# TorontoDeepLearning/convnet

Hardware: AMD Instinct MI355X
Metric: images/sec (fprop+bprop+wgrad) AlexNet 224x224 bs=256 (higher is better)
Workload: dtype f32

## Files before the change

convnet_amd/csrc/elementwise.hip:

```cpp
#include <cfloat>
#include <climits>
#include <cmath>

#include "common.h"

namespace chip {

using f32x4 = __attribute__((ext_vector_type(4))) float;

constexpr int kThreads = 256;
constexpr int kMaxBlocks = 2048;

inline int blocks_for(size_t work_items) {
  size_t b = (work_items + kThreads - 1) / kThreads;
  if (b > kMaxBlocks) b = kMaxBlocks;
  if (b < 1) b = 1;
  return (int)b;
}

template <typename F>
__global__ void map2_kernel(float* __restrict__ out, const float* a, const float* b, size_t n, bool vec, F f) {
  const size_t tid = (size_t)blockIdx.x * blockDim.x + threadIdx.x, stride = (size_t)gridDim.x * blockDim.x;
  if (vec) {
    const size_t n4 = n >> 2;
// ... 201 lines not shown
      const float b = mult * vec[(i << 2) / rows];
      f32x4 v = reinterpret_cast<const f32x4*>(mat)[i];
      v = v + b;
      reinterpret_cast<f32x4*>(out)[i] = v;
    }
  } else {
    for (size_t i = tid; i < n; i += stride) out[i] = mat[i] + mult * vec[i / rows];
  }
}

int add_row(cudamat* mat, cudamat* vec, cudamat* target, float mult) {
  if (!mat->on_device || !vec->on_device || !target->on_device) return ERROR_NOT_ON_DEVICE;
  if (mat->is_trans) return ERROR_TRANSPOSED;
  if (mat->size[1] != vec->size[1] || vec->size[0] != 1 || mat->size[0] != target->size[0] || mat->size[1] != target->size[1])
    return ERROR_INCOMPATIBLE_DIMENSIONS;
  const size_t n = numel(mat);
  const bool v4 = (mat->size[0] & 3) == 0 && aligned16(mat->data_device) && aligned16(target->data_device);
  hipLaunchKernelGGL(add_row_kernel, dim3(blocks_for(n / 4 + 1)), dim3(kThreads), 0, stream(), target->data_device, mat->data_device,
                     vec->data_device, mat->size[0], n, mult, v4);
  return launch_status();
}

__device__ __forceinline__ void sgd_one(float& g, float& w, float& h, float l2, float clip, float eps, float mom);

template <bool DO_SGD>
__global__ void rows_sq_kernel(float* __restrict__ g, float* __restrict__ w, float* __restrict__ h, int rows, int cols, int chunk,
                               float* __restrict__ partial, float l2, float clip, float eps, float mom) {
  const int r = blockIdx.x * blockDim.x + threadIdx.x;
  if (r >= rows) return;
  const int c0 = blockIdx.y * chunk, c1 = min(cols, c0 + chunk);
  float s = 0.f;
  for (int c = c0; c < c1; ++c) {
    const size_t i = (size_t)r + (size_t)rows * c;
    float wv = w[i];
    if (DO_SGD) {
      float gv = g[i], hv = h[i];
      sgd_one(gv, wv, hv, l2, clip, eps, mom);
      g[i] = gv;
      h[i] = hv;
      w[i] = wv;
    }
    s += wv * wv;
  }
  partial[(size_t)blockIdx.y * rows + r] = s;
}

template <bool DO_SGD>
__global__ void rows_sq4_kernel(float* __restrict__ g, float* __restrict__ w, float* __restrict__ h, int rows, int cols, int chunk,
                                float* __restrict__ partial, float l2, float clip, float eps, float mom) {
  const int r = 4 * (blockIdx.x * blockDim.x + threadIdx.x);
  if (r >= rows) return;
  const int c0 = blockIdx.y * chunk, c1 = min(cols, c0 + chunk);
  f32x4 s = {0.f, 0.f, 0.f, 0.f};
  auto one = [&](int c) {
    const size_t i = (size_t)r + (size_t)rows * c;
    f32x4 wv = *reinterpret_cast<f32x4*>(w + i);
    if (DO_SGD) {
      f32x4 gv = *reinterpret_cast<f32x4*>(g + i), hv = *reinterpret_cast<f32x4*>(h + i);
#pragma unroll
      for (int e = 0; e < 4; ++e) {
        float a = gv[e], b = wv[e], d = hv[e];
        sgd_one(a, b, d, l2, clip, eps, mom);
        gv[e] = a; wv[e] = b; hv[e] = d;
      }
      *reinterpret_cast<f32x4*>(g + i) = gv;
      *reinterpret_cast<f32x4*>(h + i) = hv;
      *reinterpret_cast<f32x4*>(w + i) = wv;
    }
    s += wv * wv;
  };
  int c = c0;
  for (; c + 1 < c1; c += 2) {
    one(c);
    one(c + 1);
  }
  if (c < c1) one(c);
  *reinterpret_cast<f32x4*>(partial + (size_t)blockIdx.y * rows + r) = s;
}

__global__ void row_factor_kernel(const float* __restrict__ partial, int nchunks, int rows, float norm, int constraint, float* __restrict__ factor) {
  __shared__ float sh[4][64];
  const int r = blockIdx.x * 64 + (threadIdx.x & 63), q = threadIdx.x >> 6;
  float s = 0.f;
  if (r < rows)
    for (int k = q; k < nchunks; k += 4) s += partial[(size_t)k * rows + r];
  sh[q][threadIdx.x & 63] = s;
  __syncthreads();
  if (q != 0 || r >= rows) return;
  s = sqrtf((sh[0][threadIdx.x] + sh[1][threadIdx.x]) + (sh[2][threadIdx.x] + sh[3][threadIdx.x]));
  factor[r] = (constraint == 1 || s > norm) ? norm / s : 1.f;
}

__global__ void row_scale_kernel(const float* __restrict__ src, float* __restrict__ dst, int rows, int cols, int chunk, const float* __restrict__ factor) {
  const int r = blockIdx.x * blockDim.x + threadIdx.x;
  const float f = r < rows ? factor[r] : 1.f;
  const bool in_place = src == dst;
  if (in_place && !__syncthreads_or(f != 1.f)) return;
  if (r >= rows) return;
  const int c0 = blockIdx.y * chunk, c1 = min(cols, c0 + chunk);
  for (int c = c0; c < c1; ++c) {
    const size_t i = (size_t)r + (size_t)rows * c;
    dst[i] = src[i] * f;
  }
}

inline int rows_normlimit(float* g, float* w_in, float* w_out, float* h, int rows, int cols, float norm, int constraint, bool do_sgd,
                          float l2, float clip, float eps, float mom) {
  int chunk = 64;
  while ((long)divup(rows, 256) * divup(cols, chunk) > 4096 && chunk < cols) chunk *= 2;
  const int nchunks = divup(cols, chunk);
  float* partial = static_cast<float*>(workspace(sizeof(float) * ((size_t)nchunks * rows + rows)));
  float* factor = partial + (size_t)nchunks * rows;
  dim3 grid(divup(rows, 256), nchunks);
  const bool v4 = (rows & 3) == 0 && aligned16(w_in) && (!do_sgd || (aligned16(g) && aligned16(h)));
  KernelTimer timer(do_sgd ? "rows_sq_kernel<sgd> + row_scale_kernel" : "rows_sq_kernel + row_scale_kernel", do_sgd ? "sgd_normlimit" : "normlimit", 0.0,
                    4.0 * (double)rows * cols * (do_sgd ? 7 : 3));
  if (v4) {
    const dim3 g4(divup(rows / 4, 64), nchunks);
    if (do_sgd)
      hipLaunchKernelGGL(rows_sq4_kernel<true>, g4, dim3(64), 0, stream(), g, w_in, h, rows, cols, chunk, partial, l2, clip, eps, mom);
    else
      hipLaunchKernelGGL(rows_sq4_kernel<false>, g4, dim3(64), 0, stream(), nullptr, w_in, nullptr, rows, cols, chunk, partial, 0.f, 0.f, 0.f, 0.f);
  } else if (do_sgd)
    hipLaunchKernelGGL(rows_sq_kernel<true>, grid, dim3(256), 0, stream(), g, w_in, h, rows, cols, chunk, partial, l2, clip, eps, mom);
  else
    hipLaunchKernelGGL(rows_sq_kernel<false>, grid, dim3(256), 0, stream(), nullptr, w_in, nullptr, rows, cols, chunk, partial, 0.f, 0.f, 0.f, 0.f);
  hipLaunchKernelGGL(row_factor_kernel, dim3(divup(rows, 64)), dim3(256), 0, stream(), partial, nchunks, rows, norm, constraint, factor);
  hipLaunchKernelGGL(row_scale_kernel, grid, dim3(256), 0, stream(), w_in, w_out, rows, cols, chunk, factor);
  return launch_status();
// ... 918 lines not shown
```

convnet_amd/csrc/gather_gemm.hip:

```cpp
#include <algorithm>
#include <array>
#include <cmath>
#include <map>
#include <vector>
#include <cstdlib>
#include <string>
#include <type_traits>

#include "common.h"

#include "gather_gemm.h"

namespace chip {

template <int WR, int WC, int MT, int CW, bool A_KCONTIG, bool VEC, bool O3 = false, bool SPLIT = false>
__global__ __launch_bounds__(WR* WC * 64, (O3 ? 3 : 2)) void gg_kernel(const GGParams pin, const GGClassTable ct) {
  constexpr int NT = WR * WC * 64;
  constexpr int NTC = CW / 32, CW4 = CW / 4;
  using fvec = __attribute__((ext_vector_type(NTC))) float;
  constexpr int ROWS = WR * MT * 32;
  constexpr int APITCH = A_KCONTIG ? (BK + 4) : ROWS;
  constexpr int A_STAGE = A_KCONTIG ? ROWS * APITCH : BK * ROWS;
  constexpr int B_STAGE = WC * BK * CW;
  constexpr int NA = ((A_KCONTIG ? ROWS * (BK / 4) : BK * (ROWS / 4)) + NT - 1) / NT;
// ... 733 lines not shown
#pragma unroll
    for (int t = 0; t < MT; ++t) a[0][t] = ar[lh * ROWS + t * 32];
    b4[0] = *reinterpret_cast<const fvec*>(bs + lh * BROW);
    static_for<0, BK / 2>([&](auto KK) __attribute__((always_inline)) {
      constexpr int kk = decltype(KK)::value;
      constexpr int cur = kk & 1, nxt = cur ^ 1;
      if constexpr (kk + 1 < BK / 2) {
        const int krow = 2 * (kk + 1) + lh;
#pragma unroll
        for (int t = 0; t < MT; ++t) a[nxt][t] = ar[krow * ROWS + t * 32];
        b4[nxt] = *reinterpret_cast<const fvec*>(bs + krow * BROW);
      }
      __builtin_amdgcn_sched_barrier(0);
#pragma unroll
      for (int t = 0; t < MT; ++t)
#pragma unroll
        for (int u = 0; u < NTC; ++u)
          acc[t][u] = __builtin_amdgcn_mfma_f32_32x32x2f32(a[cur][t], b4[cur][u], acc[t][u], 0, 0, 0);
    });
    stage = stage == ST - 1 ? 0 : stage + 1;
    __syncthreads();
  }

  if (tsplit >= 0) {
    float* pp = p.tail_partial + ((size_t)(L - p.tail_first) * p.tail_splits + tsplit) * (size_t)(ROWS * WC * CW);
#pragma unroll
    for (int t = 0; t < MT; ++t)
#pragma unroll
      for (int reg = 0; reg < 16; ++reg) {
        fvec v;
#pragma unroll
        for (int u = 0; u < NTC; ++u) v[u] = acc[t][u][reg];
        *reinterpret_cast<fvec*>(pp + ((size_t)(t * 16 + reg) * NC + tid) * NTC) = v;
      }
    return;
  }
  gg_epilogue<WR, WC, MT, CW, true>(p, acc, row_tile, col_tile, split, T.ncols, T.GX, T.G, T.dy0, T.dx0);
}

__global__ void gg_reduce_kernel(float* __restrict__ dst, const float* __restrict__ partial, const float* __restrict__ bias,
                                 size_t total, size_t slab, int splits, size_t per_row, float scaleTargets, int relu,
                                 const float* __restrict__ mask, float post_scale) {
  for (size_t i = (size_t)blockIdx.x * blockDim.x + threadIdx.x; i < total; i += (size_t)gridDim.x * blockDim.x) {
    float s = 0.f;
    for (int k = 0; k < splits; ++k) s += partial[(size_t)k * slab + i];
    if (scaleTargets != 0.f) s = scaleTargets * dst[i] + s;
    if (bias) s += bias[i / per_row];
    if (relu) s = s > 0.f ? s : 0.f;
    if (mask) s = mask[i] > 0.f ? s * post_scale : 0.f;
    dst[i] = s;
  }
}

__global__ void dgrad_filter_kernel(const float* __restrict__ W, float* __restrict__ Wt, int F, int C, int Ky, int Kx, int cy,
                                    int cx, int sy, int sx, int TYc, int TXc, int tap_major) {
  const size_t total = (size_t)C * TXc * TYc * F;
  for (size_t i = (size_t)blockIdx.x * blockDim.x + threadIdx.x; i < total; i += (size_t)gridDim.x * blockDim.x) {
    const int c = i % C;
    size_t r = i / C;
    int a, b, f;
    if (tap_major) {
      const int f16 = r % 16;
      r /= 16;
      const int tap = r % (TXc * TYc);
      const int fb = r / (TXc * TYc);
      f = fb * 16 + f16;
      a = tap / TXc;
      b = tap - a * TXc;
    } else {
      b = r % TXc;
      r /= TXc;
      a = r % TYc;
      f = r / TYc;
    }
    Wt[i] = W[(size_t)f + (size_t)F * ((cx + sx * b) + Kx * ((cy + sy * a) + Ky * c))];
  }
}

__global__ void filter_tapmajor_kernel(const float* __restrict__ W, float* __restrict__ Wt, int F, int C, int TYX) {
  const size_t total = (size_t)F * C * TYX;
  for (size_t i = (size_t)blockIdx.x * blockDim.x + threadIdx.x; i < total; i += (size_t)gridDim.x * blockDim.x) {
    const int f = i % F;
    size_t r = i / F;
    const int c16 = r % 16;
    r /= 16;
    const int tap = r % TYX;
    const int c = (int)(r / TYX) * 16 + c16;
    Wt[i] = W[(size_t)f + (size_t)F * (tap + (size_t)TYX * c)];
  }
}

template <int WM, int WN, int MT, int NTL, bool VEC, int TS, bool SPLIT = false>
__global__ __launch_bounds__(WM* WN * 64) void wg_kernel(const WGParams p) {
  constexpr int NT = WM * WN * 64;
  constexpr int KT = WM * MT * TS;
  constexpr int FT = WN * NTL * TS;
  constexpr int LH = 64 / TS;
  using facc = __attribute__((ext_vector_type(TS == 32 ? 16 : 4))) float;
  constexpr int PITCH = VEC ? WG_NB : WG_PITCH;
  constexpr int A_STAGE = KT * PITCH, B_STAGE = FT * PITCH;
  constexpr int NA = (KT * 8 + NT - 1) / NT, NB = (FT * 8 + NT - 1) / NT;
  extern __shared__ __attribute__((aligned(16))) float smem[];
  float* As = smem;
  float* Bs = smem + 2 * A_STAGE;

  const int tiles = p.k_tiles * p.f_tiles;
// ... 250 lines not shown
        if (fin) {
          v = v * p.scaleOutput;
          if (p.scaleTargets != 0.f) v = p.scaleTargets * ld4(dp) + v;
        }
        st4(dp, v);
      }
      return;
    }
  }
#pragma unroll
  for (int u = 0; u < NTL; ++u) {
    const int f = f0 + (wn * NTL + u) * TS + li;
    if (f >= p.F) continue;
#pragma unroll
    for (int t = 0; t < MT; ++t) {
#pragma unroll
      for (int reg = 0; reg < (TS == 32 ? 16 : 4); ++reg) {
        const int k = kc0 + (wm * MT + t) * TS + (TS == 32 ? (reg & 3) + 8 * (reg >> 2) + 4 * lh : 4 * lh + reg);
        if (k >= KB) continue;
        float* dp = (fin && k == p.K) ? p.bias_dst + f : out + (size_t)k * p.F + f;
        float v = acc[t][u][reg];
        if (fin) {
          v *= p.scaleOutput;
          if (p.scaleTargets != 0.f) v = p.scaleTargets * (*dp) + v;
        }
        *dp = v;
      }
    }
  }
}

__global__ void wg_reduce_group_kernel(float* __restrict__ stage, const float* __restrict__ partial, size_t total, int splits, int per) {
  const int g = blockIdx.y;
  const int k0 = g * per, k1 = min(splits, k0 + per);
  for (size_t i = (size_t)blockIdx.x * blockDim.x + threadIdx.x; i < total; i += (size_t)gridDim.x * blockDim.x) {
    float s = 0.f;
    for (int k = k0; k < k1; ++k) s += partial[(size_t)k * total + i];
    stage[(size_t)g * total + i] = s;
  }
}

__global__ void wg_reduce_kernel(float* __restrict__ dst, float* __restrict__ dst2, const float* __restrict__ partial, size_t total,
                                 size_t main, int splits, float scaleTargets, float scaleOutput) {
  for (size_t i = (size_t)blockIdx.x * blockDim.x + threadIdx.x; i < total; i += (size_t)gridDim.x * blockDim.x) {
    float s = 0.f;
    for (int k = 0; k < splits; ++k) s += partial[(size_t)k * total + i];
    s *= scaleOutput;
    float* d = i < main ? dst + i : dst2 + (i - main);
    if (scaleTargets != 0.f) s = scaleTargets * (*d) + s;
    *d = s;
  }
}

__global__ void __launch_bounds__(256) dot_generic_kernel(const float* __restrict__ a, const float* __restrict__ b, float* __restrict__ c, int m, int n,
                                                          int k, int ld1, int ld2, int t1, int t2, float beta, float alpha) {
  __shared__ float As[32][33], Bs[32][33];
  const int tx = threadIdx.x & 31, ty = threadIdx.x >> 5;
  const int i0 = blockIdx.x * 32, j0 = blockIdx.y * 32;
  float acc[4] = {0.f, 0.f, 0.f, 0.f};
  for (int l0 = 0; l0 < k; l0 += 32) {
    for (int r = ty; r < 32; r += 8) {
      if (t1) {
        const int i = i0 + r, l = l0 + tx;
        As[tx][r] = (i < m && l < k) ? a[(size_t)l + (size_t)ld1 * i] : 0.f;
      } else {
        const int i = i0 + tx, l = l0 + r;
        As[r][tx] = (i < m && l < k) ? a[(size_t)i + (size_t)ld1 * l] : 0.f;
      }
      if (t2) {
        const int j = j0 + tx, l = l0 + r;
        Bs[r][tx] = (j < n && l < k) ? b[(size_t)j + (size_t)ld2 * l] : 0.f;
      } else {
        const int j = j0 + r, l = l0 + tx;
        Bs[tx][r] = (j < n && l < k) ? b[(size_t)l + (size_t)ld2 * j] : 0.f;
      }
    }
    __syncthreads();
#pragma unroll 8
    for (int l = 0; l < 32; ++l) {
      const float av = As[l][tx];
#pragma unroll
      for (int q = 0; q < 4; ++q) acc[q] = fmaf(av, Bs[l][ty + 8 * q], acc[q]);
    }
    __syncthreads();
  }
  const int i = i0 + tx;
  if (i < m) {
#pragma unroll
    for (int q = 0; q < 4; ++q) {
      const int j = j0 + ty + 8 * q;
      if (j < n) {
        float* d = c + (size_t)i + (size_t)m * j;
        *d = (beta != 0.f ? beta * (*d) : 0.f) + alpha * acc[q];
      }
    }
  }
}

namespace {

constexpr int kTargetBlocks = 512;

struct GGTimer {
  const char* op;
  double flops, exec;
};
// ... 159 lines not shown
  int slots = o3 ? 768 : kTargetBlocks;
  if constexpr (kHasProducer<WC, CW, AK>) {
    if (p.KC > 0) slots = ggp_slots<WR, WC, MT, CW>(gg_split_mode(), p.apre != 0);
  }
  const double block_rate = gg_split_mode() ? 190e12 / slots : 64.0 * 4 * 2.2e9 * 0.8 / 2;
  const double flops = 2.0 * ROWS * (WC * (double)CW) * (double)p.K;
  const bool may_tail = dst_elems > 0 && gg_partial_last_round(tiles, slots, kchunks) && !CHIP_DIAG_KNOB("CONVNET_GG_NO_TAIL_SPLIT", 0);
  double best_t = 1e30;
  int splits = gg_split_k(tiles, slots, flops, block_rate, dst_elems, kchunks, kchunks, &best_t);
  int tail_s_instead = 0;
  if (splits > 1 && may_tail) {
    const int full = (tiles / slots) * slots, rem = tiles - full;
    const double t_round = flops / block_rate, tile_bytes = sizeof(float) * (double)ROWS * WC * CW;
    for (int s = 2; s <= 8 && kchunks / s >= 8; ++s) {
      const double t = (full / (double)slots + std::ceil(rem * (double)s / (double)slots) / s) * t_round + rem * (s + 1.0) * tile_bytes / 4.0e12 + 6e-6;
      if (t < best_t) {
        splits = 1;
        tail_s_instead = s;
        break;
      }
    }
  }
  p.chunks_per_split = kchunks > 0 ? divup(kchunks, splits) : 1;
  splits = kchunks > 0 ? divup(kchunks, p.chunks_per_split) : 1;
  p.splits = splits;
  p.slab = dst_elems;
  p.partial = splits > 1 ? static_cast<float*>(workspace(sizeof(float) * dst_elems * splits)) : nullptr;
  p.tail_splits = 1;
  p.tail_partial = nullptr;
  if (splits == 1 && may_tail) {
    int best_s = gg_tail_split(tiles, slots, flops, block_rate, TILE, kchunks);
    if (best_s == 1 && tail_s_instead > 1) best_s = tail_s_instead;
    if (best_s > 1) gg_set_tail(p, tiles, slots, kchunks, best_s, TILE);
  }
  dim3 grid(p.tail_splits > 1 ? 8 * (p.tail_tf8 + p.tail_tt8) : ((tiles + 7) / 8) * 8, splits);
  gg_launch_variant<WR, WC, MT, CW, AK>(p, kNoClasses, vec, o3, grid, lds_pad, tm);
  if (p.tail_splits > 1) {
    const int rem = tiles - p.tail_first;
    KernelTimer timer("gg_tail_fix_kernel", tm.op, 0.0, sizeof(float) * (double)rem * (p.tail_splits + 1) * ROWS * WC * CW);
    if (vec) hipLaunchKernelGGL((gg_tail_fix_kernel<WR, WC, MT, CW, true>), dim3(rem * kTailFixParts), dim3(WR * WC * 64), 0, stream(), p);
    else hipLaunchKernelGGL((gg_tail_fix_kernel<WR, WC, MT, CW, false>), dim3(rem * kTailFixParts), dim3(WR * WC * 64), 0, stream(), p);
  }
  if (splits > 1) gg_reduce_launch(p, dst_elems, splits, tm.op);
}

}

void wg_reduce_launch(const WGParams& p, size_t total, int splits, int groups, const char* op) {
  KernelTimer timer("wg_reduce_kernel", op, 0.0, sizeof(float) * (double)total * (splits + 1));
  size_t nb = (total + 255) / 256;
  if (nb > 4096) nb = 4096;
  const float* slabs = p.partial;
  int nslabs = splits;
  if (groups > 1) {
    float* stage = p.partial + (size_t)splits * total;
    const int per = divup(splits, groups);
    hipLaunchKernelGGL(wg_reduce_group_kernel, dim3((unsigned)nb, divup(splits, per)), dim3(256), 0, stream(), stage, p.partial, total, splits, per);
    slabs = stage;
    nslabs = divup(splits, per);
  }
  hipLaunchKernelGGL(wg_reduce_kernel, dim3((unsigned)nb), dim3(256), 0, stream(), p.dst, p.bias_dst, slabs, total, (size_t)p.K * p.F, nslabs,
                     p.scaleTargets, p.scaleOutput);
}

namespace {
struct WGBatch {
  int frames = 0, frame = 0, splits = 0;
  size_t total = 0;
  void* (*arena)(size_t) = nullptr;
  size_t max_bytes = 0;
  WGParams last;
};
WGBatch g_wgb;
}
void wg_batch_begin(int frames, void* (*slab_arena)(size_t), size_t max_bytes) {
  g_wgb = WGBatch{};
  g_wgb.frames = frames;
  g_wgb.arena = slab_arena;
  g_wgb.max_bytes = max_bytes;
}
bool wg_batch_active() { return g_wgb.frames > 0; }
int wg_batch_frame() { return g_wgb.frame; }
float* wg_batch_partial(const WGParams& p, size_t total, int splits) {
  WGBatch& b = g_wgb;
  if (!b.frames) return nullptr;
  CHIP_REQUIRE(b.frame < b.frames);
  const size_t S = (size_t)b.frames * splits;
  const size_t bytes = sizeof(float) * total * (S + (S > 64 ? 32 : 0));
  if (b.frame == 0) {
    if (bytes > b.max_bytes) {
      b.frames = 0;
      return nullptr;
    }
    b.splits = splits;
    b.total = total;
  }
  CHIP_REQUIRE(b.splits == splits && b.total == total);
  float* arena = static_cast<float*>(b.arena(bytes));
  b.last = p;
  b.last.partial = arena;
  return arena + (size_t)b.frame++ * splits * total;
}
void wg_batch_end() {
  WGBatch& b = g_wgb;
  if (b.frames && b.frame > 0) {
    CHIP_REQUIRE(b.frame == b.frames);
    const int S = b.frames * b.splits;
    wg_reduce_launch(b.last, b.total, S, S > 64 ? 32 : 1, "conv_wgrad");
  }
  b.frames = 0;
}

void gg_reduce_launch(const GGParams& p, size_t dst_elems, int splits, const char* op) {
  KernelTimer timer("gg_reduce_kernel", op, 0.0, sizeof(float) * (double)dst_elems * (splits + 1));
  size_t nb = (dst_elems + 255) / 256;
  if (nb > 4096) nb = 4096;
  hipLaunchKernelGGL(gg_reduce_kernel, dim3((unsigned)nb), dim3(256), 0, stream(), p.dst, p.partial, p.bias, dst_elems, p.slab, splits,
                     (size_t)p.DP * p.N, p.scaleTargets, p.relu, p.mask, p.post_scale);
}

namespace {

template <bool AK>
void gg_run(GGParams& p, bool vec, size_t dst_elems, const GGTimer& tm) {
  gg_with_tile(gg_tile(p.R, vec, p.skinny != 0), [&](auto t) {
    using T = decltype(t);
    gg_launch_cfg<T::WR, T::WC, T::MT, T::CW, AK>(p, vec, dst_elems, tm);
  });
}

void gg_run_classes(GGParams& p, GGClassTable& ct, bool vec, const GGTimer& tm) {
  gg_with_tile(gg_tile(p.R, vec, false), [&](auto t) {
    using T = decltype(t);
    gg_launch_classes<T::WR, T::WC, T::MT, T::CW>(p, ct, vec, tm);
  });
}

template <int WM, int WN, int MT, int NTL, int TS = 32>
void wg_launch_cfg(WGParams& p, bool vec, const GGTimer& tm) {
  constexpr int KT = WM * MT * TS, FT = WN * NTL * TS;
  const size_t lds = sizeof(float) * 2 * (KT + FT) * (vec ? WG_NB : WG_PITCH);
  p.k_tiles = divup(p.K, KT);
  if (p.bias_dst && divup(p.K + 1, KT) != p.k_tiles) p.bias_dst = nullptr;
  p.f_tiles = divup(p.F, FT);
  p.zero = zero_page();
  p.prio = wg_prio_mode();
  const int tiles = p.k_tiles * p.f_tiles;
  const size_t total = (size_t)(p.K + (p.bias_dst ? 1 : 0)) * p.F;
  const bool no_wide = CHIP_DIAG_KNOB("CONVNET_WG_NO_WIDE", 0) != 0;
  p.wide = (!no_wide && vec && TS == 32 && WM == 2 && WN == 2 && MT == 2 && NTL == 2 && p.F % 4 == 0 && aligned16(p.dst) &&
            (!p.bias_dst || aligned16(p.bias_dst))) ? 1 : 0;
  int splits = 1;
  if (tiles < kTargetBlocks) {
    splits = kTargetBlocks / tiles;
    const int max_by_len = p.chunks_total / 16 > 0 ? p.chunks_total / 16 : 1;
    if (splits > max_by_len) splits = max_by_len;
    const size_t max_by_bytes = (size_t(256) << 20) / (total * sizeof(float)) + 1;
    if ((size_t)splits > max_by_bytes) splits = (int)max_by_bytes;
    if (splits > 1024) splits = 1024;
    if (splits < 1) splits = 1;
  }
  p.chunks_per_split = divup(p.chunks_total, splits);
  splits = divup(p.chunks_total, p.chunks_per_split);
  p.splits = splits;
  const int groups = splits > 64 ? 32 : 1;
  float* const frame_slabs = wg_batch_partial(p, total, splits);
  p.partial = frame_slabs ? frame_slabs
                          : splits > 1 ? static_cast<float*>(workspace(sizeof(float) * total * (splits + (groups > 1 ? groups : 0)))) : nullptr;
  dim3 grid(((tiles * splits + 7) / 8) * 8), block(WM * WN * 64);
  static const std::string kname_f = "wg_kernel<" + std::to_string(WM) + "," + std::to_string(WN) + "," + std::to_string(MT) + "," + std::to_string(NTL) + (TS == 16 ? ",x16>" : ">");
  static const std::string kname_s = kname_f.substr(0, kname_f.size() - 1) + ",split>";
// ... 451 lines not shown
```

convnet_amd/csrc/pool_norm.hip:

```cpp
#include <cfloat>
#include <cstdlib>
#include <mutex>
#include <utility>

#include "common.h"

namespace chip {

using f32x4 = __attribute__((ext_vector_type(4))) float;

struct PoolGeo {
  int N, C, H, W, Ky, Kx, sy, sx, py, px, My, Mx;
  int nvec;
  int xper, xtotal, xrows, xbx;
};

__device__ __forceinline__ bool pool_block(const PoolGeo& g, int& bx, int& row, int& c) {
  if (g.xper == 0) {
    bx = blockIdx.x; row = blockIdx.y; c = blockIdx.z;
    return true;
  }
  const int b = blockIdx.x, slot = b >> 3;
  const int L = (b & 7) * g.xper + slot;
  if (slot >= g.xper || L >= g.xtotal) return false;
// ... 310 lines not shown
using u32x2 = __attribute__((ext_vector_type(2))) unsigned;

__global__ void __launch_bounds__(256) pool_fwd_max32_mask_kernel(const float* __restrict__ in, float* __restrict__ out, u32x2* __restrict__ mask, PoolGeo g) {
  int bx, by, c;
  if (!pool_block(g, bx, by, c)) return;
  const int MB = (g.Mx + 1) >> 1;
  const int j = bx * 256 + threadIdx.x;
  if (j >= MB * g.nvec) return;
  const int xb = j / g.nvec, n = 4 * (j - xb * g.nvec);
  const int oy0 = 2 * by, ox0 = 2 * xb;
  const int ys = oy0 * 2 + g.py, xs = ox0 * 2 + g.px;
  const float* plane = in + (size_t)c * g.H * g.W * g.N + n;
  f32x4 v[5][5];
  bool ok[5][5];
#pragma unroll
  for (int dy = 0; dy < 5; ++dy)
#pragma unroll
    for (int dx = 0; dx < 5; ++dx) {
      const int y = ys + dy, x = xs + dx;
      ok[dy][dx] = y >= 0 && y < g.H && x >= 0 && x < g.W;
      const size_t o = ok[dy][dx] ? ((size_t)y * g.W + x) * g.N : 0;
      v[dy][dx] = *reinterpret_cast<const f32x4*>(plane + o);
    }
#pragma unroll
  for (int a = 0; a < 2; ++a)
#pragma unroll
    for (int b = 0; b < 2; ++b) {
      const int oy = oy0 + a, ox = ox0 + b;
      if (oy >= g.My || ox >= g.Mx) continue;
      f32x4 acc = {-FLT_MAX, -FLT_MAX, -FLT_MAX, -FLT_MAX};
#pragma unroll
      for (int dy = 0; dy < 3; ++dy)
#pragma unroll
        for (int dx = 0; dx < 3; ++dx)
#pragma unroll
          for (int e = 0; e < 4; ++e)
            acc[e] = (ok[2 * a + dy][2 * b + dx] && acc[e] < v[2 * a + dy][2 * b + dx][e]) ? v[2 * a + dy][2 * b + dx][e] : acc[e];
      unsigned m[4];
#pragma unroll
      for (int e = 0; e < 4; ++e) {
        m[e] = acc[e] > 0.f ? 1u << 9 : 0u;
#pragma unroll
        for (int dy = 0; dy < 3; ++dy)
#pragma unroll
          for (int dx = 0; dx < 3; ++dx)
            m[e] |= (ok[2 * a + dy][2 * b + dx] && v[2 * a + dy][2 * b + dx][e] == acc[e]) ? 1u << (3 * dy + dx) : 0u;
      }
      const size_t o = ((size_t)(c * g.My + oy) * g.Mx + ox) * g.N + n;
      *reinterpret_cast<f32x4*>(out + o) = acc;
      mask[o >> 2] = u32x2{m[0] | (m[1] << 16), m[2] | (m[3] << 16)};
    }
}

__global__ void __launch_bounds__(256) pool_undo_max32_mask_kernel(const float* __restrict__ grads, const u32x2* __restrict__ mask, float* __restrict__ out,
                                                                   PoolGeo g, float st, bool relu) {
  int bx, by, c;
  if (!pool_block(g, bx, by, c)) return;
  const int WB = (g.W + 1) >> 1;
  const int j = bx * 256 + threadIdx.x;
  if (j >= WB * g.nvec) return;
  const int xb = j / g.nvec, n = 4 * (j - xb * g.nvec);
  const int iy0 = 2 * by, ix0 = 2 * xb;
  const int ty0 = iy0 - g.py, tx0 = ix0 - g.px;
  const int oy0 = (ty0 + 1) / 2 - 1, ox0 = (tx0 + 1) / 2 - 1;
  const size_t pplane = (size_t)c * g.My * g.Mx * g.N + n;
  f32x4 gv[2][2];
  unsigned mk[2][2][4];
  bool pok[2][2];
  const unsigned need = relu ? 1u << 9 : 0u;
#pragma unroll
  for (int a = 0; a < 2; ++a)
#pragma unroll
    for (int b = 0; b < 2; ++b) {
      const int oy = oy0 + a, ox = ox0 + b;
      pok[a][b] = oy >= 0 && oy < g.My && ox >= 0 && ox < g.Mx;
      const size_t o = pplane + (pok[a][b] ? ((size_t)oy * g.Mx + ox) * g.N : 0);
      gv[a][b] = *reinterpret_cast<const f32x4*>(grads + o);
      const u32x2 w = mask[o >> 2];
      const unsigned m4[4] = {w[0] & 0xffffu, w[0] >> 16, w[1] & 0xffffu, w[1] >> 16};
#pragma unroll
      for (int e = 0; e < 4; ++e) mk[a][b][e] = (m4[e] & need) == need ? m4[e] : 0u;
    }
#pragma unroll
  for (int dy = 0; dy < 2; ++dy)
#pragma unroll
    for (int dx = 0; dx < 2; ++dx) {
      if (!(iy0 + dy < g.H && ix0 + dx < g.W)) continue;
      const int ty = ty0 + dy, tx = tx0 + dx;
      f32x4 acc = {0.f, 0.f, 0.f, 0.f};
#pragma unroll
      for (int a = 0; a < 2; ++a)
#pragma unroll
        for (int b = 0; b < 2; ++b) {
          const int oy = oy0 + a, ox = ox0 + b;
          const bool cov = pok[a][b] && 2 * oy <= ty && ty < 2 * oy + 3 && 2 * ox <= tx && tx < 2 * ox + 3;
          const unsigned bit = cov ? 1u << (3 * (ty - 2 * oy) + (tx - 2 * ox)) : 0u;
#pragma unroll
          for (int e = 0; e < 4; ++e) acc[e] += (mk[a][b][e] & bit) ? gv[a][b][e] : 0.f;
        }
      float* op = out + ((size_t)(c * g.H + iy0 + dy) * g.W + ix0 + dx) * g.N + n;
      if (st != 0.f) acc = st * *reinterpret_cast<const f32x4*>(op) + acc;
      *reinterpret_cast<f32x4*>(op) = acc;
    }
}

__device__ __forceinline__ void win_fwd(int j, int C, int sizeF, bool blocked, int& start, int& end) {
  start = blocked ? (j / sizeF) * sizeF : -sizeF / 2 + j;
  end = min(C, start + sizeF);
  start = max(0, start);
}
__device__ __forceinline__ void win_bwd(int j, int C, int sizeF, bool blocked, int& start, int& end) {
  start = blocked ? (j / sizeF) * sizeF : -sizeF + sizeF / 2 + j + 1;
  end = min(C, start + sizeF);
  start = max(0, start);
}

__device__ __forceinline__ float sq_rn(float v) {
#pragma clang fp contract(off)
  return v * v;
}
__device__ __forceinline__ f32x4 sq_rn(f32x4 v) {
#pragma clang fp contract(off)
  return v * v;
}

__global__ void rnorm_fwd_kernel(const float* __restrict__ in, float* __restrict__ out, size_t locs, int C, int sizeF, float addScale,
                                 float powScale, bool blocked, bool vec, int cseg, int nseg, bool relu) {
  const size_t nq = (locs + 3) >> 2;
  for (size_t q = (size_t)blockIdx.x * blockDim.x + threadIdx.x; q < nq * nseg; q += (size_t)gridDim.x * blockDim.x) {
    const int seg = (int)(q / nq);
    const size_t l = (q % nq) << 2;
    const int j0 = seg * cseg, j1 = min(C, j0 + cseg);
    const int rem = (int)min((size_t)4, locs - l);
    f32x4 sum = {0.f, 0.f, 0.f, 0.f};
    int ps, pe;
    {
      int e0;
      win_fwd(j0, C, sizeF, blocked, ps, e0);
      pe = ps;
    }
    for (int j = j0; j < j1; ++j) {
      int s, e;
      win_fwd(j, C, sizeF, blocked, s, e);
      for (int i = ps; i < s; ++i) {
        const f32x4 v = ldv(in + (size_t)i * locs + l, 0, rem, vec);
        sum = sum - sq_rn(v);
      }
      for (int i = pe; i < e; ++i) {
        const f32x4 v = ldv(in + (size_t)i * locs + l, 0, rem, vec);
        sum = sum + sq_rn(v);
      }
      const f32x4 x = ldv(in + (size_t)j * locs + l, 0, rem, vec);
      f32x4 y;
#pragma unroll
      for (int t = 0; t < 4; ++t) {
// ... 793 lines not shown
static bool park_pool_undo(cudamat* images, cudamat* maxGrads, cudamat* maxActs, cudamat* targets, Shape4D* images_shape, Shape4D* maxGrads_shape,
                           const ConvDesc& d, float scaleTargets) {
  if (!defer_begin(3, launch_pool_undo)) return false;
  PendingOp& o = pending();
  o.m[0] = *images; o.m[1] = *maxGrads; o.m[2] = *maxActs; o.m[3] = *targets;
  o.s[0] = *images_shape; o.s[1] = *maxGrads_shape;
  o.desc = d;
  o.scaleTargets = scaleTargets;
  return true;
}
void MaxPoolUndoGemm(cudamat* images, cudamat* maxGrads, cudamat* maxActs, cudamat* targets, Shape4D* images_shape, Shape4D* maxGrads_shape,
                     ConvDesc d, float scaleTargets) {
  if (park_pool_undo(images, maxGrads, maxActs, targets, images_shape, maxGrads_shape, d, scaleTargets)) return;
  pool_undo<true>(images, maxGrads, maxActs, targets, images_shape, maxGrads_shape, d, scaleTargets);
}
void MaxPoolUndoRelu(cudamat* images, cudamat* maxGrads, cudamat* maxActs, cudamat* targets, Shape4D* images_shape,
                     Shape4D* maxGrads_shape, ConvDesc d, float scaleTargets) {
  pool_undo<true>(images, maxGrads, maxActs, targets, images_shape, maxGrads_shape, d, scaleTargets, true);
}
void MaxPoolUndo(cudamat* images, cudamat* maxGrads, cudamat* maxActs, cudamat* targets, Shape4D* images_shape, Shape4D* maxGrads_shape,
                 ConvDesc d, float scaleTargets) {
  if (park_pool_undo(images, maxGrads, maxActs, targets, images_shape, maxGrads_shape, d, scaleTargets)) return;
  pool_undo<true>(images, maxGrads, maxActs, targets, images_shape, maxGrads_shape, d, scaleTargets);
}
static bool mask_geo_ok(const PoolGeo& g, const cudamat* images, const cudamat* pooled_a, const cudamat* pooled_b, const cudamat* mask) {
  const bool vec = g.N % 4 == 0 && a16(images->data_device) && a16(pooled_a->data_device) && (!pooled_b || a16(pooled_b->data_device)) &&
                   a16(mask->data_device);
  return fixed_window(g, vec) == 32 && g.py <= 0 && g.px <= 0 && numel(mask) * 2 >= (size_t)g.N * g.C * g.My * g.Mx;
}
int MaxPoolMask(cudamat* images, cudamat* targets, cudamat* mask, Shape4D* images_shape, Shape4D* targets_shape, ConvDesc conv_desc) {
  if (!images->on_device || !targets->on_device || !mask->on_device) return ERROR_NOT_ON_DEVICE;
  Pool3DGeo g3;
  if (pool_time_geo(images_shape, targets_shape, conv_desc, images, targets, g3)) return ERROR_UNSUPPORTED;
  PoolGeo g = pool_geo(images_shape, targets_shape, conv_desc, images, targets);
  if (!mask_geo_ok(g, images, targets, nullptr, mask)) return ERROR_UNSUPPORTED;
  KernelTimer timer("pool_fwd_mask_kernel<max>", "pool_fwd", 0.0, (double)g.N * g.C * (4.0 * g.H * g.W + 6.0 * g.My * g.Mx));
  const int hb = (g.My + 1) / 2;
  dim3 bgrid(divup(((g.Mx + 1) / 2) * g.nvec, 256), hb, g.C);
  bgrid = pool_xcd_grid(g, bgrid.x, hb, bgrid);
  hipLaunchKernelGGL(pool_fwd_max32_mask_kernel, bgrid, dim3(256), 0, stream(), images->data_device, targets->data_device,
                     reinterpret_cast<u32x2*>(mask->data_device), g);
  return launch_status();
}
int MaxPoolUndoMask(cudamat* maxGrads, cudamat* mask, cudamat* targets, Shape4D* targets_shape, Shape4D* maxGrads_shape, ConvDesc conv_desc,
                    float scaleTargets, int relu) {
  if (!maxGrads->on_device || !targets->on_device || !mask->on_device) return ERROR_NOT_ON_DEVICE;
  if (relu && scaleTargets != 0.f) return ERROR_UNSUPPORTED;
  Pool3DGeo g3;
  if (pool_time_geo(targets_shape, maxGrads_shape, conv_desc, targets, maxGrads, g3)) return ERROR_UNSUPPORTED;
  PoolGeo g = pool_geo(targets_shape, maxGrads_shape, conv_desc, targets, maxGrads);
  if (!mask_geo_ok(g, targets, maxGrads, nullptr, mask)) return ERROR_UNSUPPORTED;
  KernelTimer timer("pool_undo_mask_kernel<max>", "pool_undo", 0.0,
                    (double)g.N * g.C * ((scaleTargets != 0.f ? 8.0 : 4.0) * g.H * g.W + 6.0 * g.My * g.Mx));
  const int hb = (g.H + 1) / 2;
  dim3 bgrid(divup(((g.W + 1) / 2) * g.nvec, 256), hb, g.C);
  bgrid = pool_xcd_grid(g, bgrid.x, hb, bgrid);
  hipLaunchKernelGGL(pool_undo_max32_mask_kernel, bgrid, dim3(256), 0, stream(), maxGrads->data_device,
                     reinterpret_cast<const u32x2*>(mask->data_device), targets->data_device, g, scaleTargets, relu != 0);
  return launch_status();
}
void AvgPoolUndoGemm(cudamat* avgGrads, cudamat* targets, Shape4D* avgGrads_shape, Shape4D* targets_shape, ConvDesc d, float scaleTargets) {
  pool_undo<false>(nullptr, avgGrads, nullptr, targets, targets_shape, avgGrads_shape, d, scaleTargets);
}
void AvgPoolUndo(cudamat* avgGrads, cudamat* targets, Shape4D* avgGrads_shape, Shape4D* targets_shape, ConvDesc d, float scaleTargets) {
  pool_undo<false>(nullptr, avgGrads, nullptr, targets, targets_shape, avgGrads_shape, d, scaleTargets);
}

static void rnorm_fwd_impl(cudamat* images, cudamat* targets, int numFilters, int sizeF, float addScale, float powScale, bool blocked, bool relu) {
  const size_t total = numel(images);
  CHIP_REQUIRE(numel(targets) == total && numFilters > 0 && total % numFilters == 0 && sizeF > 0);
  const size_t locs = total / numFilters;
  const bool vec = locs % 4 == 0 && a16(images->data_device) && a16(targets->data_device);
  KernelTimer timer("rnorm_fwd_kernel", "rnorm_fwd", 0.0, 8.0 * total);
  {
    const int C = numFilters;
    int LT = C <= 192 ? 64 : (C <= 384 ? 32 : (C <= 768 ? 16 : 0));
    if (const int f = CHIP_DIAG_KNOB("CONVNET_RNORM_FWD_LT", 0)) LT = f;
    if (rnorm_fwd_fast(images->data_device, targets->data_device, locs, C, sizeF, addScale, powScale, blocked, vec, relu)) return;
    if (LT) {
      const size_t smem = sizeof(float) * (size_t)C * LT;
      const bool xcd = !CHIP_DIAG_KNOB("CONVNET_RNORM_NO_XCD", 0);
      const unsigned tiles = (unsigned)((locs + LT - 1) / LT);
      const dim3 grid(xcd ? (tiles + 7) / 8 * 8 : tiles), block(256);
#define RN_FWD(L) hipLaunchKernelGGL(rnorm_fwd_lds_kernel<L>, grid, block, smem, stream(), images->data_device, targets->data_device, locs, C, sizeF, addScale, powScale, blocked, vec, relu, tiles, xcd)
      if (LT == 64) RN_FWD(64);
      else if (LT == 32) RN_FWD(32);
      else if (LT == 16) RN_FWD(16);
      else RN_FWD(8);
#undef RN_FWD
      return;
    }
  }
  CHIP_REQUIRE(images->data_device != targets->data_device);
  int cseg, nseg;
  rnorm_segments((locs + 3) / 4, numFilters, sizeF, cseg, nseg);
  hipLaunchKernelGGL(rnorm_fwd_kernel, dim3(grid_for((locs + 3) / 4 * nseg)), dim3(256), 0, stream(), images->data_device, targets->data_device, locs,
                     numFilters, sizeF, addScale, powScale, blocked, vec, cseg, nseg, relu);
}
static void launch_rnorm_fwd(PendingOp& o) { rnorm_fwd_impl(&o.m[0], &o.m[1], o.i0, o.i1, o.f0, o.f1, o.b0, o.relu != 0); }
void ResponseNormCrossMapGemm(cudamat* images, cudamat* targets, int numFilters, int sizeF, float addScale, float powScale, bool blocked) {
  if (defer_begin(4, launch_rnorm_fwd)) {
    PendingOp& o = pending();
    o.m[0] = *images; o.m[1] = *targets;
    o.i0 = numFilters; o.i1 = sizeF; o.f0 = addScale; o.f1 = powScale; o.b0 = blocked;
    return;
  }
  rnorm_fwd_impl(images, targets, numFilters, sizeF, addScale, powScale, blocked, false);
}
void ResponseNormCrossMapRelu(cudamat* images, cudamat* targets, int numFilters, int sizeF, float addScale, float powScale, bool blocked) {
  rnorm_fwd_impl(images, targets, numFilters, sizeF, addScale, powScale, blocked, true);
}
// ... 57 lines not shown
```

Baseline: 28340.

## Vectorize split-K reductions, batch SGD loads, and enlarge max-pool undo tiles

Adds float4-vectorized variants of the split-K output and weight-gradient reduction kernels, with one thread per four elements instead of grid-stride scalar loops. The row-norm SGD kernel now issues four columns of loads before computing and writes gradient and history with nontemporal stores. The max-pool undo kernel is templated to handle 4x4 input tiles per thread with compile-time parity offsets, so overlapping pooled gradients and masks are loaded once per tile and the coverage tests are resolved at compile time. The cost is more register pressure and extra template instantiations, and the vector paths depend on alignment checks at launch.

```diff
diff --git a/convnet_amd/csrc/elementwise.hip b/convnet_amd/csrc/elementwise.hip
--- a/convnet_amd/csrc/elementwise.hip
+++ b/convnet_amd/csrc/elementwise.hip
@@ -277,29 +277,40 @@
   if (r >= rows) return;
   const int c0 = blockIdx.y * chunk, c1 = min(cols, c0 + chunk);
   f32x4 s = {0.f, 0.f, 0.f, 0.f};
-  auto one = [&](int c) {
-    const size_t i = (size_t)r + (size_t)rows * c;
-    f32x4 wv = *reinterpret_cast<f32x4*>(w + i);
+  constexpr int NC = 4;
+  auto finish = [&](size_t i, f32x4 gv, f32x4 wv, f32x4 hv) {
     if (DO_SGD) {
-      f32x4 gv = *reinterpret_cast<f32x4*>(g + i), hv = *reinterpret_cast<f32x4*>(h + i);
 #pragma unroll
       for (int e = 0; e < 4; ++e) {
         float a = gv[e], b = wv[e], d = hv[e];
         sgd_one(a, b, d, l2, clip, eps, mom);
         gv[e] = a; wv[e] = b; hv[e] = d;
       }
-      *reinterpret_cast<f32x4*>(g + i) = gv;
-      *reinterpret_cast<f32x4*>(h + i) = hv;
+      __builtin_nontemporal_store(gv, reinterpret_cast<f32x4*>(g + i));
+      __builtin_nontemporal_store(hv, reinterpret_cast<f32x4*>(h + i));
       *reinterpret_cast<f32x4*>(w + i) = wv;
     }
     s += wv * wv;
   };
+  const f32x4 zero = {0.f, 0.f, 0.f, 0.f};
   int c = c0;
-  for (; c + 1 < c1; c += 2) {
-    one(c);
-    one(c + 1);
-  }
-  if (c < c1) one(c);
+  for (; c + NC <= c1; c += NC) {
+    f32x4 gv[NC], wv[NC], hv[NC];
+#pragma unroll
+    for (int k = 0; k < NC; ++k) {
+      const size_t i = (size_t)r + (size_t)rows * (c + k);
+      wv[k] = *reinterpret_cast<f32x4*>(w + i);
+      gv[k] = DO_SGD ? *reinterpret_cast<f32x4*>(g + i) : zero;
+      hv[k] = DO_SGD ? *reinterpret_cast<f32x4*>(h + i) : zero;
+    }
+#pragma unroll
+    for (int k = 0; k < NC; ++k) finish((size_t)r + (size_t)rows * (c + k), gv[k], wv[k], hv[k]);
+  }
+  for (; c < c1; ++c) {
+    const size_t i = (size_t)r + (size_t)rows * c;
+    const f32x4 wv = *reinterpret_cast<f32x4*>(w + i);
+    finish(i, DO_SGD ? *reinterpret_cast<f32x4*>(g + i) : zero, wv, DO_SGD ? *reinterpret_cast<f32x4*>(h + i) : zero);
+  }
   *reinterpret_cast<f32x4*>(partial + (size_t)blockIdx.y * rows + r) = s;
 }
 
diff --git a/convnet_amd/csrc/gather_gemm.hip b/convnet_amd/csrc/gather_gemm.hip
--- a/convnet_amd/csrc/gather_gemm.hip
+++ b/convnet_amd/csrc/gather_gemm.hip
@@ -809,6 +809,43 @@
   }
 }
 
+__device__ __forceinline__ f32x4 slab_sum4(const float* __restrict__ partial, size_t slab, int k0, int k1) {
+  f32x4 s = {0.f, 0.f, 0.f, 0.f};
+  int k = k0;
+  for (; k + 4 <= k1; k += 4) {
+    const f32x4 a = *reinterpret_cast<const f32x4*>(partial + (size_t)k * slab), b = *reinterpret_cast<const f32x4*>(partial + (size_t)(k + 1) * slab),
+                c = *reinterpret_cast<const f32x4*>(partial + (size_t)(k + 2) * slab), d = *reinterpret_cast<const f32x4*>(partial + (size_t)(k + 3) * slab);
+    s += a;
+    s += b;
+    s += c;
+    s += d;
+  }
+  for (; k < k1; ++k) s += *reinterpret_cast<const f32x4*>(partial + (size_t)k * slab);
+  return s;
+}
+
+__global__ void __launch_bounds__(256) gg_reduce4_kernel(float* __restrict__ dst, const float* __restrict__ partial, const float* __restrict__ bias,
+                                                         size_t total, size_t slab, int splits, size_t per_row, float scaleTargets, int relu,
+                                                         const float* __restrict__ mask, float post_scale) {
+  const size_t i = 4 * ((size_t)blockIdx.x * blockDim.x + threadIdx.x);
+  if (i >= total) return;
+  f32x4 v = slab_sum4(partial + i, slab, 0, splits);
+  f32x4 old = {0.f, 0.f, 0.f, 0.f}, mk = {0.f, 0.f, 0.f, 0.f};
+  if (scaleTargets != 0.f) old = *reinterpret_cast<const f32x4*>(dst + i);
+  if (mask) mk = *reinterpret_cast<const f32x4*>(mask + i);
+  const float b = bias ? bias[i / per_row] : 0.f;
+#pragma unroll
+  for (int e = 0; e < 4; ++e) {
+    float s = v[e];
+    if (scaleTargets != 0.f) s = __builtin_fmaf(scaleTargets, old[e], s);
+    if (bias) s += b;
+    if (relu) s = s > 0.f ? s : 0.f;
+    if (mask) s = mk[e] > 0.f ? s * post_scale : 0.f;
+    v[e] = s;
+  }
+  *reinterpret_cast<f32x4*>(dst + i) = v;
+}
+
 __global__ void dgrad_filter_kernel(const float* __restrict__ W, float* __restrict__ Wt, int F, int C, int Ky, int Kx, int cy,
                                     int cx, int sy, int sx, int TYc, int TXc, int tap_major) {
   const size_t total = (size_t)C * TXc * TYc * F;
@@ -1165,6 +1202,30 @@
   }
 }
 
+__global__ void __launch_bounds__(256) wg_reduce_group4_kernel(float* __restrict__ stage, const float* __restrict__ partial, size_t total, int splits, int per) {
+  const int g = blockIdx.y;
+  const size_t i = 4 * ((size_t)blockIdx.x * blockDim.x + threadIdx.x);
+  if (i >= total) return;
+  *reinterpret_cast<f32x4*>(stage + (size_t)g * total + i) = slab_sum4(partial + i, total, g * per, min(splits, g * per + per));
+}
+__global__ void __launch_bounds__(256) wg_reduce4_kernel(float* __restrict__ dst, float* __restrict__ dst2, const float* __restrict__ partial, size_t total,
+                                                         size_t main, int splits, float scaleTargets, float scaleOutput) {
+  const size_t i = 4 * ((size_t)blockIdx.x * blockDim.x + threadIdx.x);
+  if (i >= total) return;
+  f32x4 v = slab_sum4(partial + i, total, 0, splits);
+  float* d = i < main ? dst + i : dst2 + (i - main);
+  f32x4 old = {0.f, 0.f, 0.f, 0.f};
+  if (scaleTargets != 0.f) old = *reinterpret_cast<const f32x4*>(d);
+#pragma unroll
+  for (int e = 0; e < 4; ++e) {
+    float s = v[e];
+    s *= scaleOutput;
+    if (scaleTargets != 0.f) s = __builtin_fmaf(scaleTargets, old[e], s);
+    v[e] = s;
+  }
+  *reinterpret_cast<f32x4*>(d) = v;
+}
+
 __global__ void __launch_bounds__(256) dot_generic_kernel(const float* __restrict__ a, const float* __restrict__ b, float* __restrict__ c, int m, int n,
                                                           int k, int ld1, int ld2, int t1, int t2, float beta, float alpha) {
   __shared__ float As[32][33], Bs[32][33];
@@ -1430,15 +1491,24 @@
   if (nb > 4096) nb = 4096;
   const float* slabs = p.partial;
   int nslabs = splits;
+  const size_t main = (size_t)p.K * p.F;
+  const bool v4 = total % 4 == 0 && main % 4 == 0 && aligned16(p.partial) && aligned16(p.dst) && (main == total || aligned16(p.bias_dst));
+  const unsigned nb4 = (unsigned)((total / 4 + 255) / 256);
   if (groups > 1) {
     float* stage = p.partial + (size_t)splits * total;
     const int per = divup(splits, groups);
-    hipLaunchKernelGGL(wg_reduce_group_kernel, dim3((unsigned)nb, divup(splits, per)), dim3(256), 0, stream(), stage, p.partial, total, splits, per);
+    if (v4)
+      hipLaunchKernelGGL(wg_reduce_group4_kernel, dim3(nb4, divup(splits, per)), dim3(256), 0, stream(), stage, p.partial, total, splits, per);
+    else
+      hipLaunchKernelGGL(wg_reduce_group_kernel, dim3((unsigned)nb, divup(splits, per)), dim3(256), 0, stream(), stage, p.partial, total, splits, per);
     slabs = stage;
     nslabs = divup(splits, per);
   }
-  hipLaunchKernelGGL(wg_reduce_kernel, dim3((unsigned)nb), dim3(256), 0, stream(), p.dst, p.bias_dst, slabs, total, (size_t)p.K * p.F, nslabs,
-                     p.scaleTargets, p.scaleOutput);
+  if (v4)
+    hipLaunchKernelGGL(wg_reduce4_kernel, dim3(nb4), dim3(256), 0, stream(), p.dst, p.bias_dst, slabs, total, main, nslabs, p.scaleTargets, p.scaleOutput);
+  else
+    hipLaunchKernelGGL(wg_reduce_kernel, dim3((unsigned)nb), dim3(256), 0, stream(), p.dst, p.bias_dst, slabs, total, main, nslabs, p.scaleTargets,
+                       p.scaleOutput);
 }
 
 namespace {
@@ -1493,8 +1563,13 @@
   KernelTimer timer("gg_reduce_kernel", op, 0.0, sizeof(float) * (double)dst_elems * (splits + 1));
   size_t nb = (dst_elems + 255) / 256;
   if (nb > 4096) nb = 4096;
-  hipLaunchKernelGGL(gg_reduce_kernel, dim3((unsigned)nb), dim3(256), 0, stream(), p.dst, p.partial, p.bias, dst_elems, p.slab, splits,
-                     (size_t)p.DP * p.N, p.scaleTargets, p.relu, p.mask, p.post_scale);
+  const size_t per_row = (size_t)p.DP * p.N;
+  if (dst_elems % 4 == 0 && p.slab % 4 == 0 && per_row % 4 == 0 && aligned16(p.dst) && aligned16(p.partial) && aligned16(p.mask))
+    hipLaunchKernelGGL(gg_reduce4_kernel, dim3((unsigned)((dst_elems / 4 + 255) / 256)), dim3(256), 0, stream(), p.dst, p.partial, p.bias, dst_elems,
+                       p.slab, splits, per_row, p.scaleTargets, p.relu, p.mask, p.post_scale);
+  else
+    hipLaunchKernelGGL(gg_reduce_kernel, dim3((unsigned)nb), dim3(256), 0, stream(), p.dst, p.partial, p.bias, dst_elems, p.slab, splits, per_row,
+                       p.scaleTargets, p.relu, p.mask, p.post_scale);
 }
 
 namespace {
diff --git a/convnet_amd/csrc/pool_norm.hip b/convnet_amd/csrc/pool_norm.hip
--- a/convnet_amd/csrc/pool_norm.hip
+++ b/convnet_amd/csrc/pool_norm.hip
@@ -386,55 +386,54 @@
     }
 }
 
+template <int BY, int BX, int PY, int PX>
 __global__ void __launch_bounds__(256) pool_undo_max32_mask_kernel(const float* __restrict__ grads, const u32x2* __restrict__ mask, float* __restrict__ out,
                                                                    PoolGeo g, float st, bool relu) {
+  constexpr int NA = BY / 2 + 1, NB = BX / 2 + 1;
   int bx, by, c;
   if (!pool_block(g, bx, by, c)) return;
-  const int WB = (g.W + 1) >> 1;
+  const int WB = (g.W + BX - 1) / BX;
   const int j = bx * 256 + threadIdx.x;
   if (j >= WB * g.nvec) return;
   const int xb = j / g.nvec, n = 4 * (j - xb * g.nvec);
-  const int iy0 = 2 * by, ix0 = 2 * xb;
+  const int iy0 = BY * by, ix0 = BX * xb;
   const int ty0 = iy0 - g.py, tx0 = ix0 - g.px;
   const int oy0 = (ty0 + 1) / 2 - 1, ox0 = (tx0 + 1) / 2 - 1;
   const size_t pplane = (size_t)c * g.My * g.Mx * g.N + n;
-  f32x4 gv[2][2];
-  unsigned mk[2][2][4];
-  bool pok[2][2];
+  f32x4 gv[NA][NB];
+  unsigned mk[NA][NB][4];
   const unsigned need = relu ? 1u << 9 : 0u;
 #pragma unroll
-  for (int a = 0; a < 2; ++a)
-#pragma unroll
-    for (int b = 0; b < 2; ++b) {
+  for (int a = 0; a < NA; ++a)
+#pragma unroll
+    for (int b = 0; b < NB; ++b) {
       const int oy = oy0 + a, ox = ox0 + b;
-      pok[a][b] = oy >= 0 && oy < g.My && ox >= 0 && ox < g.Mx;
-      const size_t o = pplane + (pok[a][b] ? ((size_t)oy * g.Mx + ox) * g.N : 0);
+      const bool pok = oy >= 0 && oy < g.My && ox >= 0 && ox < g.Mx;
+      const size_t o = pplane + (pok ? ((size_t)oy * g.Mx + ox) * g.N : 0);
       gv[a][b] = *reinterpret_cast<const f32x4*>(grads + o);
       const u32x2 w = mask[o >> 2];
       const unsigned m4[4] = {w[0] & 0xffffu, w[0] >> 16, w[1] & 0xffffu, w[1] >> 16};
 #pragma unroll
-      for (int e = 0; e < 4; ++e) mk[a][b][e] = (m4[e] & need) == need ? m4[e] : 0u;
-    }
-#pragma unroll
-  for (int dy = 0; dy < 2; ++dy)
-#pragma unroll
-    for (int dx = 0; dx < 2; ++dx) {
+      for (int e = 0; e < 4; ++e) mk[a][b][e] = (pok && (m4[e] & need) == need) ? m4[e] : 0u;
+    }
+#pragma unroll
+  for (int dy = 0; dy < BY; ++dy)
+#pragma unroll
+    for (int dx = 0; dx < BX; ++dx) {
       if (!(iy0 + dy < g.H && ix0 + dx < g.W)) continue;
-      const int ty = ty0 + dy, tx = tx0 + dx;
+      const int uy = dy + 2 - PY, ux = dx + 2 - PX;
       f32x4 acc = {0.f, 0.f, 0.f, 0.f};
 #pragma unroll
-      for (int a = 0; a < 2; ++a)
-#pragma unroll
-        for (int b = 0; b < 2; ++b) {
-          const int oy = oy0 + a, ox = ox0 + b;
-          const bool cov = pok[a][b] && 2 * oy <= ty && ty < 2 * oy + 3 && 2 * ox <= tx && tx < 2 * ox + 3;
-          const unsigned bit = cov ? 1u << (3 * (ty - 2 * oy) + (tx - 2 * ox)) : 0u;
+      for (int a = (uy - 1) / 2; a <= uy / 2; ++a)
+#pragma unroll
+        for (int b = (ux - 1) / 2; b <= ux / 2; ++b) {
+          const unsigned bit = 1u << (3 * (uy - 2 * a) + (ux - 2 * b));
 #pragma unroll
           for (int e = 0; e < 4; ++e) acc[e] += (mk[a][b][e] & bit) ? gv[a][b][e] : 0.f;
         }
       float* op = out + ((size_t)(c * g.H + iy0 + dy) * g.W + ix0 + dx) * g.N + n;
       if (st != 0.f) acc = st * *reinterpret_cast<const f32x4*>(op) + acc;
-      *reinterpret_cast<f32x4*>(op) = acc;
+      __builtin_nontemporal_store(acc, reinterpret_cast<f32x4*>(op));
     }
 }
 
@@ -1334,11 +1333,20 @@
   if (!mask_geo_ok(g, targets, maxGrads, nullptr, mask)) return ERROR_UNSUPPORTED;
   KernelTimer timer("pool_undo_mask_kernel<max>", "pool_undo", 0.0,
                     (double)g.N * g.C * ((scaleTargets != 0.f ? 8.0 : 4.0) * g.H * g.W + 6.0 * g.My * g.Mx));
-  const int hb = (g.H + 1) / 2;
-  dim3 bgrid(divup(((g.W + 1) / 2) * g.nvec, 256), hb, g.C);
+  constexpr int BY = 4, BX = 4;
+  const int hb = divup(g.H, BY);
+  dim3 bgrid(divup(divup(g.W, BX) * g.nvec, 256), hb, g.C);
   bgrid = pool_xcd_grid(g, bgrid.x, hb, bgrid);
-  hipLaunchKernelGGL(pool_undo_max32_mask_kernel, bgrid, dim3(256), 0, stream(), maxGrads->data_device,
-                     reinterpret_cast<const u32x2*>(mask->data_device), targets->data_device, g, scaleTargets, relu != 0);
+  auto launch = [&](auto kernel) {
+    hipLaunchKernelGGL(kernel, bgrid, dim3(256), 0, stream(), maxGrads->data_device, reinterpret_cast<const u32x2*>(mask->data_device),
+                       targets->data_device, g, scaleTargets, relu != 0);
+  };
+  switch ((-g.py & 1) * 2 + (-g.px & 1)) {
+    case 0: launch(pool_undo_max32_mask_kernel<BY, BX, 0, 0>); break;
+    case 1: launch(pool_undo_max32_mask_kernel<BY, BX, 0, 1>); break;
+    case 2: launch(pool_undo_max32_mask_kernel<BY, BX, 1, 0>); break;
+    default: launch(pool_undo_max32_mask_kernel<BY, BX, 1, 1>); break;
+  }
   return launch_status();
 }
 void AvgPoolUndoGemm(cudamat* avgGrads, cudamat* targets, Shape4D* avgGrads_shape, Shape4D* targets_shape, ConvDesc d, float scaleTargets) {
```

Measured after the change: 28650, median of 6. 1.01x the previous value.
